# ChristophReich1996/Multi-StyleGAN

Measured on AMD Instinct MI355X. Metric: training images/sec (G+D step, 256^2, seq=3x2ch), higher is better.
Workload: dtype bf16

## Files before the change

### multi_stylegan_amd/csrc/conv_upconv.hip

```cpp
#include "conv_dispatch.h"
#include <stdlib.h>

typedef __bf16 bf16v8 __attribute__((ext_vector_type(8)));
typedef const __attribute__((address_space(1))) char* gptr_t;
typedef __attribute__((address_space(3))) char* lds_t;

struct UpconvParams {
    int B, H, W, Cx, N, O, ldy;
    long long x_bstride, w_bstride, y_bstride;
    int m_tiles, xcd_samples;
};

constexpr int UC_M = 128, UC_K = 512, UC_ROW = UC_K * 2;
constexpr int UC_PATCH = 32 * 64 * 2;

constexpr int UC_WAVES = 8;

__global__ __launch_bounds__(64 * UC_WAVES, 1) void conv_upconv_kernel(const bf16_t* __restrict__ x, const bf16_t* __restrict__ w,
                                                             bf16_t* __restrict__ y, UpconvParams p) {
    __shared__ __attribute__((aligned(16))) char smem[UC_M * UC_ROW + UC_WAVES * UC_PATCH];
    const int tid = threadIdx.x, lane = tid & 63, wid = tid >> 6;
    const int wid_u = __builtin_amdgcn_readfirstlane(wid);
    const int lr = lane & 31, lh = lane >> 5;
    int b, tile;
    if (p.xcd_samples) {
        const int xcd = blockIdx.x & 7, k = blockIdx.x >> 3;
        const int j = k / p.m_tiles;
        tile = k - j * p.m_tiles;
        b = xcd + 8 * j;
    } else {
        b = blockIdx.x / p.m_tiles;
        tile = blockIdx.x - b * p.m_tiles;
    }
    b = __builtin_amdgcn_readfirstlane(b);
    tile = __builtin_amdgcn_readfirstlane(tile);
    const int m0 = tile * UC_M;
    const int hw = p.H * p.W;

    {
        const gptr_t xb = (gptr_t)(x + (long long)b * p.x_bstride);
#pragma unroll 4
        for (int j = 0; j < UC_M / UC_WAVES; ++j) {
            const int r = wid_u * (UC_M / UC_WAVES) + j;
            const int m = m0 + r < hw ? m0 + r : 0;
            const gptr_t src = xb + ((long long)m * p.Cx + ((lane ^ (r & 15)) << 3)) * 2;
            __builtin_amdgcn_global_load_lds(src, (lds_t)(smem + r * UC_ROW), 16, 0, 0);
        }
        asm volatile("s_waitcnt vmcnt(0)" ::: "memory");
        __syncthreads();
    }

    const bf16_t* wb = w + (long long)b * p.w_bstride;
    bf16_t* yb = y + (long long)b * p.y_bstride;
    char* patch = smem + UC_M * UC_ROW + wid * UC_PATCH;
    const int swz = lr & 15;
    const int n_slices = p.N / 64;

    for (int slice = wid_u; slice < n_slices; slice += UC_WAVES) {
        const int n0 = slice * 64;
        f32x16 acc[4][2];
#pragma unroll
        for (int i = 0; i < 4; ++i)
#pragma unroll
            for (int j = 0; j < 2; ++j)
#pragma unroll
                for (int e = 0; e < 16; ++e) acc[i][j][e] = 0.f;

        const bf16_t* wrow[2] = {wb + (long long)(n0 + lr) * UC_K + 32 * lh, wb + (long long)(n0 + 32 + lr) * UC_K + 32 * lh};
        bf16v8 fb[2][2][4];
#pragma unroll
        for (int j = 0; j < 2; ++j)
#pragma unroll
            for (int u = 0; u < 4; ++u) fb[0][j][u] = *reinterpret_cast<const bf16v8*>(wrow[j] + 8 * u);
        bf16v8 fa[4];
        auto read_a = [&](int step, int i) __attribute__((always_inline)) {
            const int slot = ((8 * (step >> 2) + 4 * lh + (step & 3)) ^ swz) << 4;
            fa[i] = *reinterpret_cast<const bf16v8*>(smem + (32 * i + lr) * UC_ROW + slot);
        };
#pragma unroll
        for (int i = 0; i < 4; ++i) read_a(0, i);
#pragma unroll
        for (int t = 0; t < UC_K / 64; ++t) {
            if (t + 1 < UC_K / 64) {
#pragma unroll
                for (int j = 0; j < 2; ++j)
#pragma unroll
                    for (int u = 0; u < 4; ++u)
// ... 18 lines not shown
#pragma unroll
        for (int i = 0; i < 4; ++i) {
#pragma unroll
            for (int j = 0; j < 2; ++j)
#pragma unroll
                for (int g = 0; g < 4; ++g) {
                    const int unit = 8 * j + 2 * g + lh;
                    uint2 pk;
                    pk.x = (unsigned)f2bf(acc[i][j][4 * g + 0]) | ((unsigned)f2bf(acc[i][j][4 * g + 1]) << 16);
                    pk.y = (unsigned)f2bf(acc[i][j][4 * g + 2]) | ((unsigned)f2bf(acc[i][j][4 * g + 3]) << 16);
                    *reinterpret_cast<uint2*>(patch + lr * 128 + ((unit ^ (lr & 15)) << 3)) = pk;
                }
            asm volatile("s_waitcnt lgkmcnt(0)" ::: "memory");
            u32x4 v[4];
#pragma unroll
            for (int pass = 0; pass < 4; ++pass) {
                const int row = pass * 8 + er;
                v[pass] = *reinterpret_cast<const u32x4*>(patch + row * 128 + ((ec ^ ((row & 15) >> 1)) << 4));
                if (row & 1) v[pass] = u32x4{v[pass][2], v[pass][3], v[pass][0], v[pass][1]};
            }
#pragma unroll
            for (int pass = 0; pass < 4; ++pass) {
                const int m = m0 + 32 * i + pass * 8 + er;
                if (m < hw) {
                    const int oh = m / p.W, ow = m - oh * p.W;
                    const long long pix = (long long)(2 * oh + dy) * (2 * p.W) + 2 * ow + dx;
                    *reinterpret_cast<u32x4*>(yb + pix * p.ldy + c0 + ec * 8) = v[pass];
                }
            }
            asm volatile("s_waitcnt lgkmcnt(0)" ::: "memory");
        }
    }
}

bool conv_upconv_eligible(const ConvProblem& q, const ActEpilogue* act, bool has_bias, ConvPlan* plan) {
    static const int enabled = msg_tunable("MSG_CONV_UPCONV", 1);
    if (q.dtype != MSG_BF16 || has_bias || conv_act_mode(act)) return false;
    if (!enabled || !q.pixel_shuffle || !q.per_sample() || q.kh != 1 || q.kw != 1 || q.stride != 1 || q.pad != 0 || q.in_up != 1)
        return false;
    if (q.Cx != UC_K || q.Ck != UC_K || q.N % 256 || (q.N / 4) % 64 || q.IH != q.OH || q.IW != q.OW) return false;
    const long long hw = (long long)q.OH * q.OW, m_tiles = (hw + UC_M - 1) / UC_M;
    if (hw < 16384 || hw >= (1ll << 30)) return false;
    if (m_tiles * q.B < 256 || m_tiles * q.B >= (1ll << 31)) return false;
    if (q.w_batch_stride < (long long)q.N * UC_K) return false;
    *plan = ConvPlan{CONV_UPCONV, UC_M, q.N, true};
    return true;
}

void conv_upconv_launch(const ConvProblem& q, const ConvPlan&, const void* x, const void* w, void* y, void* stream) {
    UpconvParams p{};
    p.B = q.B; p.H = q.OH; p.W = q.OW; p.Cx = q.Cx; p.N = q.N; p.O = q.N / 4; p.ldy = q.ldy;
    p.x_bstride = q.x_bstride();
    p.w_bstride = q.w_batch_stride;
    p.y_bstride = q.y_bstride();
    p.m_tiles = (int)(((long long)q.OH * q.OW + UC_M - 1) / UC_M);
    static const int xcd_order = msg_tunable("MSG_UPCONV_XCD", 1);
    p.xcd_samples = xcd_order && q.B % 8 == 0;
    dim3 grid((unsigned)((long long)p.m_tiles * q.B));
    hipLaunchKernelGGL(conv_upconv_kernel, grid, dim3(64 * UC_WAVES), 0, (hipStream_t)stream, (const bf16_t*)x, (const bf16_t*)w,
                       (bf16_t*)y, p);
}
```

### include/msg_hip.h

```cpp
#ifndef MSG_HIP_H
#define MSG_HIP_H

#ifdef __cplusplus
extern "C" {
#endif

enum { MSG_OK = 0, MSG_EINVAL = -1, MSG_EUNSUPPORTED = -2, MSG_ELAUNCH = -3 };
enum { MSG_F32 = 0, MSG_BF16 = 1, MSG_F16 = 2, MSG_F64 = 3, MSG_F32_SPLIT = 4 };

#define MSG_ABI_VERSION 5
int msg_abi_version(void);
const char* msg_build_arch(void);
const char* msg_strerror(int code);

int msg_upfirdn2d(const void* x, const float* fir, void* y, int dtype,
                  int major, int in_h, int in_w, int minor, int kh, int kw,
                  int up_x, int up_y, int down_x, int down_y,
                  int pad_x0, int pad_x1, int pad_y0, int pad_y1, void* stream);

int msg_upfirdn2d_pitched(const void* x, const float* fir, void* y, int dtype,
                          int major, int in_h, int in_w, int minor, int in_pitch, int kh, int kw,
                          int up_x, int up_y, int down_x, int down_y,
                          int pad_x0, int pad_x1, int pad_y0, int pad_y1, void* stream);

// ... 155 lines not shown
long long msg_act_pointwise_head_backward_workspace(long long npix, int C);
int msg_act_pointwise_head_backward(const void* x, const float* bias, const float* w, const float* gy, void* gx,
                                    float* grad_bias_and_w, int dtype, long long npix, int C, float wscale,
                                    float alpha, float scale, float* ws, long long ws_floats, void* stream);

int msg_linear_fprop(const float* x, const float* w, const float* bias, float* y, int M, int N, int K,
                     float gain, float bias_gain, void* stream);
int msg_linear_dgrad(const float* gy, const float* w, float* gx, int M, int N, int K, float gain, void* stream);
int msg_linear_wgrad(const float* gy, const float* x, float* gw, float* gb, int M, int N, int K,
                     float gain, float bias_gain, void* stream);

int msg_linear_grouped_fprop(const float* x, const int* slot, const float* const* w, const float* const* bias, float* y,
                             int G, int M, int N, int K, int L, float gain, float bias_gain, void* stream);
int msg_linear_grouped_dgrad(const float* gy, const float* const* w, float* gx, int G, int M, int N, int K, float gain,
                             void* stream);
int msg_linear_grouped_wgrad(const float* gy, const float* x, const int* slot, float* gw, float* gb, int G, int M, int N,
                             int K, int L, float gain, float bias_gain, void* stream);
int msg_linear_grouped_wgrad_ptrs(const float* gy, const float* x, const int* slot, float* const* gw, float* const* gb, int G,
                                  int M, int N, int K, int L, float gain, float bias_gain, void* stream);

enum {
    MSG_PLAN_REG = 0,
    MSG_PLAN_DMA = 1,
    MSG_PLAN_PP = 2,
    MSG_PLAN_ROW3 = 3,
    MSG_PLAN_ROW3N = 4,
    MSG_PLAN_THIN = 5,
    MSG_PLAN_UPCONV = 6,
    MSG_FPLAN_FIELDS = 5
};
int msg_conv2d_fprop_launch_plan(int dtype, int B, int IH, int IW, int Cx, int Ck, int OH, int OW, int N, int ldy,
                                 int kh, int kw, int stride, int pad, int in_up, int pixel_shuffle,
                                 long long w_batch_stride, int has_bias, int epilogue, long long* out, int n_out_fields);
enum {
    MSG_WPLAN_GENERIC = 0,
    MSG_WPLAN_DMA = 1,
    MSG_WPLAN_UNI = 2,
    MSG_WPLAN_ROW3 = 3,
    MSG_WPLAN_ROW3_W32 = 4,
    MSG_WPLAN_FIELDS = 11
};
int msg_conv2d_wgrad_plan(int dtype, int B, int IH, int IW, int Cx, int I, int OH, int OW, int ldgy,
                          int O, int ldgw, int kh, int kw, int stride, int pad, int pixel_shuffle,
                          int per_sample, int k_chunks, long long* out, int n_out_fields);
int msg_conv2d_fprop_plan(int dtype, int B, int IH, int IW, int Cx, int Ck, int OH, int OW, int N,
                          int kh, int kw, long long w_batch_stride);
long long msg_conv2d_fprop_act_backward_workspace(int dtype, int B, int IH, int IW, int Cx, int Ck, int OH, int OW,
                                                  int N, int kh, int kw, long long w_batch_stride, int has_noise);
int msg_conv2d_fprop_upconv_eligible(int B, int IH, int IW, int Cx, int Ck, int OH, int OW, int N, int kh, int kw,
                                     int stride, int pad, int in_up, int pixel_shuffle, long long w_batch_stride);
int msg_conv2d_fprop_thin_eligible(int B, int IH, int IW, int Cx, int Ck, int OH, int OW, int N, int ldy, int kh, int kw,
                                   int stride, int pad, int in_up, int pixel_shuffle, int act_mode);

int msg_flat_adam(float* param, const float* grad, float* exp_avg, float* exp_avg_sq, float* ema, long long n,
                  const float* coef, float lr, float beta1, float beta2, float eps, int step, float ema_decay,
                  void* stream);
int msg_flat_ema(float* ema, const float* param, long long n, float decay, void* stream);

long long msg_tlfm_prepare_workspace(int B, int T);
int msg_tlfm_prepare(const unsigned short* raw, const unsigned char* hflip, void* out, int dtype,
                     int B, int C, int T, int H, int W, int vflip,
                     float lo1, float div1, float lo2, float div2,
                     unsigned int* ws, void* stream);

int msg_tlfm_frame_range(const unsigned short* frames, long long N, int H, int W,
                         unsigned int* range, void* stream);
// ... 34 lines not shown
```

### multi_stylegan_amd/csrc/conv_fprop.hip

```cpp
#include "conv_dispatch.h"
#include <stdlib.h>

typedef __bf16 bf16v8 __attribute__((ext_vector_type(8)));
typedef const __attribute__((address_space(1))) char* gptr_t;
typedef const __attribute__((address_space(1))) u32x4* gvec_t;
typedef __attribute__((address_space(3))) char* lds_t;

struct ConvParams {
    int B, IH, IW, Cx, Ck, OH, OW, N, ldy;
    int kh, kw, stride, pad, in_up, pixel_shuffle, per_sample;
    long long x_bstride, w_bstride, y_bstride;
    int Mtot, n_chunks, n_iters, m_tiles, n_tiles;
    ActEpilogue act;
};

constexpr int BM = 128, BN = 128, ROWB = 128;
constexpr int STAGE_BYTES = (BM + BN) * ROWB;
__device__ __attribute__((aligned(256))) unsigned int g_zero_page[16384];

__device__ __forceinline__ int swz(int row, int slot) { return row * ROWB + ((slot ^ ((row >> 1) & 7)) << 4); }

template <int SPLIT>
__device__ __forceinline__ void split_park(const u32x4& raw, char* dst) {
    uint2 pl[3];
#pragma unroll
    for (int h = 0; h < 2; ++h) {
        const float x0 = __uint_as_float(raw[2 * h]), x1 = __uint_as_float(raw[2 * h + 1]);
        const unsigned hp = (unsigned)f2bf(x0) | ((unsigned)f2bf(x1) << 16);
        const float r0 = x0 - __uint_as_float(hp << 16), r1 = x1 - __uint_as_float(hp & 0xffff0000u);
        const unsigned mp = (unsigned)f2bf(r0) | ((unsigned)f2bf(r1) << 16);
        (h ? pl[0].y : pl[0].x) = hp;
        (h ? pl[1].y : pl[1].x) = mp;
        if constexpr (SPLIT == 3) {
            const float q0 = r0 - __uint_as_float(mp << 16), q1 = r1 - __uint_as_float(mp & 0xffff0000u);
            (h ? pl[2].y : pl[2].x) = (unsigned)f2bf(q0) | ((unsigned)f2bf(q1) << 16);
        }
    }
#pragma unroll
    for (int p = 0; p < SPLIT; ++p) *reinterpret_cast<uint2*>(dst + p * 64) = pl[p];
}

template <typename T, bool DMA, int LEAN = 0, int SPLIT = 0>
__global__ __launch_bounds__(256, LEAN ? LEAN : 2) void conv_fprop_kernel(const T* __restrict__ x, const T* __restrict__ w,
                                                            T* __restrict__ y, const float* __restrict__ bias,
                                                            ConvParams p) {
    constexpr int VEC = 16 / sizeof(T);
    constexpr int BKE = ROWB / sizeof(T);
    static_assert(!LEAN || (!DMA && sizeof(T) == 2), "lean variant: bf16, register staging");
    static_assert(SPLIT == 0 || sizeof(T) == 4, "split-bf16 products are a mode of the fp32-storage kernel");
    static_assert(SPLIT == 0 || !DMA, "the split planes are written from the staging registers");
    constexpr int SROW = SPLIT ? SPLIT * 64 + 16 : ROWB;
    constexpr int STAGE = SPLIT ? (BM + BN) * SROW : STAGE_BYTES;
    constexpr bool ONE_STAGE = LEAN != 0 || SPLIT == 3;
    constexpr int SMEM_BYTES = ONE_STAGE ? (STAGE > 65536 || sizeof(T) == 2 ? STAGE : 65536) : 2 * STAGE;
    __shared__ __attribute__((aligned(16))) char smem[SMEM_BYTES];

    const int tid = threadIdx.x, lane = tid & 63, wid = tid >> 6;
    const int wm = wid >> 1, wn = wid & 1;
    const int lr = lane & 31, lh = lane >> 5;
    const unsigned L = xcd_remap(blockIdx.x, gridDim.x);
    const int n0 = (int)(L % p.n_tiles) * BN;
    const int m0 = (int)(L / p.n_tiles) * BM;
    const int bz = blockIdx.z;

    const int wid_u = __builtin_amdgcn_readfirstlane(wid);
    const int slot_phys = tid & 7;
    int row_of[4];
#pragma unroll
    for (int j = 0; j < 4; ++j) row_of[j] = DMA ? (wid * 32 + 8 * j + (lane >> 3)) : ((tid >> 3) + 32 * j);
    const int slot = DMA ? 0 : slot_phys;
    int a_ih0[4], a_iw0[4];
    long long a_boff[4];
    int a_slot[4];
    bool a_ok[4];
    const int ohw = p.OH * p.OW;
#pragma unroll
    for (int j = 0; j < 4; ++j) {
        const int m = m0 + row_of[j];
        const int slot_j = DMA ? (slot_phys ^ ((row_of[j] >> 1) & 7)) : slot_phys;
        a_ok[j] = m < p.Mtot;
        const int mm = a_ok[j] ? m : 0;
        const int b = p.per_sample ? bz : mm / ohw;
        const int pix = p.per_sample ? mm : mm - b * ohw;
        const int oh = pix / p.OW, ow = pix - oh * p.OW;
        a_ih0[j] = oh * p.stride - p.pad;
        a_iw0[j] = ow * p.stride - p.pad;
        a_boff[j] = ((long long)((DMA && p.per_sample) ? 0 : b) * p.x_bstride + slot_j * VEC +
// ... 158 lines not shown
                        for (int order = SPLIT - 1; order >= 0; --order)
#pragma unroll
                            for (int pa = 0; pa <= order; ++pa)
                                acc[i][j] = __builtin_amdgcn_mfma_f32_32x32x16_bf16(bf[order - pa][j], af[pa][i], acc[i][j], 0, 0, 0);
                    }
            }
        } else {
#pragma unroll
            for (int q = 0; q < 4; ++q) {
                f32x4 fa[2], fb[2];
#pragma unroll
                for (int t = 0; t < 2; ++t) {
                    fa[t] = *reinterpret_cast<const f32x4*>(sa + swz(wm * 64 + t * 32 + lr, 4 * lh + q));
                    fb[t] = *reinterpret_cast<const f32x4*>(sb + swz(wn * 64 + t * 32 + lr, 4 * lh + q));
                }
#pragma unroll
                for (int e = 0; e < 4; ++e)
#pragma unroll
                    for (int i = 0; i < 2; ++i)
#pragma unroll
                        for (int j = 0; j < 2; ++j)
                            acc[i][j] = __builtin_amdgcn_mfma_f32_32x32x2f32(fb[j][e], fa[i][e], acc[i][j], 0, 0, 0);
            }
        }
    };
    if constexpr (ONE_STAGE) {
        load_next();
        for (int it = 0; it < p.n_iters; ++it) {
            if (it) __syncthreads();
            park(0);
            if (it + 1 < p.n_iters) load_next();
            __syncthreads();
            mma_step(smem);
        }
    } else {
        if constexpr (DMA) {
            dma_stage = 0;
            load_next();
        } else {
            load_next();
            park(0);
            if (p.n_iters > 1) load_next();
        }
        for (int it = 0; it < p.n_iters; ++it) {
            if constexpr (DMA) asm volatile("s_waitcnt vmcnt(0)" ::: "memory");
            __syncthreads();
            if constexpr (DMA) {
                if (it + 1 < p.n_iters) { dma_stage = (it + 1) & 1; load_next(); }
            } else {
                if (it + 1 < p.n_iters) park((it + 1) & 1);
                if (it + 2 < p.n_iters) load_next();
            }
            mma_step(smem + (it & 1) * STAGE);
        }
    }
    if constexpr (DMA) asm volatile("s_waitcnt vmcnt(0)" ::: "memory");
    __syncthreads();

    constexpr int PITCH = 64 * sizeof(T);
    constexpr int UNITB = 4 * sizeof(T);
    char* ep = smem + wid * (64 * PITCH);
#pragma unroll
    for (int j = 0; j < 2; ++j)
#pragma unroll
        for (int g = 0; g < 4; ++g) {
            const int unit = 8 * j + 2 * g + lh;
// ... 83 lines not shown
    }
    T* ybase = y + (p.pixel_shuffle ? nn : n);
    if (n_ok && lim >= VEC) {
#pragma unroll
        for (int pass = 0; pass < NPASS; ++pass)
            if (gp[pass] >= 0) *reinterpret_cast<u32x4*>(ybase + (long long)gp[pass] * p.ldy) = v[pass];
    } else if (n_ok) {
#pragma unroll
        for (int pass = 0; pass < NPASS; ++pass) {
            if (gp[pass] < 0) continue;
            T tmp[VEC];
            *reinterpret_cast<u32x4*>(tmp) = v[pass];
            T* dst = ybase + (long long)gp[pass] * p.ldy;
            for (int e = 0; e < lim; ++e) dst[e] = tmp[e];
        }
    }
}

static ConvPlan conv_generic_select(const ConvProblem& q) {
    const int n_iters = q.kh * q.kw * (q.Ck / (ROWB / q.esz()));
    static const int variant = msg_tunable("MSG_CONV_VARIANT", 0);
    const bool dma = q.fits31() && (variant == 1 || (variant == 0 && n_iters >= 8));
    static const int lean_max = msg_tunable("MSG_CONV_LEAN", 4);
    ConvPlan plan{CONV_REG, BM, BN, true};
    if (q.split) plan.kernel = CONV_REG_SPLIT;
    else if (dma) plan.kernel = CONV_DMA;
    else if (q.dtype == MSG_BF16 && n_iters <= lean_max) plan.kernel = CONV_REG_LEAN;
    const long long mtot = q.mtot(), blocks = ((mtot + BM - 1) / BM) * ((q.N + BN - 1) / BN);
    plan.supported = mtot < (1ll << 31) && blocks < (1ll << 31) &&
                     (long long)(n_iters + 1) * ROWB + 128 <= 65536;
    return plan;
}

static void conv_generic_launch(const ConvProblem& q, const ConvPlan& plan, const void* x, const void* w, const float* bias, void* y,
                                const ActEpilogue* act, void* stream) {
    ConvParams p{};
    conv_fill_common(p, q, act);
    conv_fill_taps(p, q);
    p.n_chunks = q.Ck / (ROWB / q.esz());
    p.n_iters = q.kh * q.kw * p.n_chunks;
    p.m_tiles = (int)((q.mtot() + BM - 1) / BM);
    p.n_tiles = (q.N + BN - 1) / BN;
    dim3 grid((unsigned)((long long)p.m_tiles * p.n_tiles), 1, q.samples());
#define GENERIC(T, ...) hipLaunchKernelGGL((conv_fprop_kernel<T, __VA_ARGS__>), grid, dim3(256), 0, (hipStream_t)stream, \
                                           (const T*)x, (const T*)w, (T*)y, bias, p)
    const bool bf16 = q.dtype == MSG_BF16;
    if (bf16 && plan.kernel == CONV_REG_LEAN) GENERIC(bf16_t, false, 3);
    else if (bf16 && plan.kernel == CONV_DMA) GENERIC(bf16_t, true);
    else if (bf16) GENERIC(bf16_t, false);
    else if (plan.kernel == CONV_REG_SPLIT) GENERIC(float, false, 0, 3);
    else if (plan.kernel == CONV_DMA) GENERIC(float, true);
    else GENERIC(float, false);
#undef GENERIC
}

ConvPlan conv_fprop_select(const ConvProblem& q, const ActEpilogue* act, bool has_bias) {
    ConvPlan plan;
    if (conv_thin_eligible(q, act, &plan)) return plan;
    if (conv_upconv_eligible(q, act, has_bias, &plan)) return plan;
    if (conv_row3_eligible(q, act, has_bias, &plan)) return plan;
    if (conv_pp_eligible(q, &plan)) return plan;
    return conv_generic_select(q);
}

static ConvProblem conv_problem(int dtype, int B, int IH, int IW, int Cx, int Ck, int OH, int OW, int N, int ldy,
                                int kh, int kw, int stride, int pad, int in_up, int pixel_shuffle, long long w_batch_stride) {
    const int split = dtype == MSG_F32_SPLIT ? 3 : 0;
    return ConvProblem{split ? (int)MSG_F32 : dtype, split, B, IH, IW, Cx, Ck, OH, OW, N, ldy, kh, kw, stride, pad, in_up, pixel_shuffle,
                       w_batch_stride};
}

static ConvPlan fprop_select(const ConvProblem& q, int act_mode, bool has_bias) {
    ActEpilogue act{};
    act.enabled = act_mode;
    return conv_fprop_select(q, &act, has_bias);
}

static int fprop_check(const ConvProblem& q, const void* const* io) {
    if (q.B < 0 || q.IH <= 0 || q.IW <= 0 || q.OH <= 0 || q.OW <= 0 || q.N <= 0 || q.kh <= 0 || q.kw <= 0 || q.stride <= 0 ||
        q.in_up <= 0 || q.Cx <= 0 || q.Ck <= 0 || q.ldy <= 0 || (io && (!io[0] || !io[1] || !io[2])))
        return MSG_EINVAL;
    if (q.dtype != MSG_F32 && q.dtype != MSG_BF16) return MSG_EUNSUPPORTED;
    const int vec = 16 / q.esz(), bke = ROWB / q.esz();
// ... 49 lines not shown
    for (int k = 0; k < MSG_FPLAN_FIELDS && k < n_out_fields; ++k) out[k] = fields[k];
    return MSG_OK;
}

static ConvProblem conv_query_problem(int dtype, int B, int IH, int IW, int Cx, int Ck, int OH, int OW, int N, int kh, int kw,
                                      long long w_batch_stride) {
    return conv_problem(dtype, B, IH, IW, Cx, Ck, OH, OW, N, N <= 8 ? 8 : (N + 7) / 8 * 8, kh, kw, 1, kh / 2, 1, 0, w_batch_stride);
}
extern "C" int msg_conv2d_fprop_plan(int dtype, int B, int IH, int IW, int Cx, int Ck, int OH, int OW, int N,
                                     int kh, int kw, long long w_batch_stride) {
    return plan_code(fprop_select(conv_query_problem(dtype, B, IH, IW, Cx, Ck, OH, OW, N, kh, kw, w_batch_stride), 0, false).kernel);
}
extern "C" long long msg_conv2d_fprop_act_backward_workspace(int dtype, int B, int IH, int IW, int Cx, int Ck, int OH, int OW,
                                                             int N, int kh, int kw, long long w_batch_stride, int has_noise) {
    const ConvProblem q = conv_query_problem(dtype, B, IH, IW, Cx, Ck, OH, OW, N, kh, kw, w_batch_stride);
    long long rows, entries;
    act_backward_partials(q, fprop_select(q, 3, false), &rows, &entries);
    return rows ? rows * N + (has_noise ? entries : 0) : 0;
}
extern "C" int msg_conv2d_fprop_upconv_eligible(int B, int IH, int IW, int Cx, int Ck, int OH, int OW, int N, int kh, int kw,
                                                int stride, int pad, int in_up, int pixel_shuffle, long long w_batch_stride) {
    return fprop_select(conv_problem(MSG_BF16, B, IH, IW, Cx, Ck, OH, OW, N, N / 4, kh, kw, stride, pad, in_up, pixel_shuffle,
                                     w_batch_stride), 0, false).kernel == CONV_UPCONV;
}
extern "C" int msg_conv2d_fprop_thin_eligible(int B, int IH, int IW, int Cx, int Ck, int OH, int OW, int N, int ldy,
                                              int kh, int kw, int stride, int pad, int in_up, int pixel_shuffle,
                                              int act_mode) {
    const ConvKernel kernel = fprop_select(conv_problem(MSG_BF16, B, IH, IW, Cx, Ck, OH, OW, N, ldy, kh, kw, stride, pad, in_up,
                                                        pixel_shuffle, 0), act_mode, false).kernel;
    return kernel == CONV_THIN_N ? 1 : kernel == CONV_THIN_K ? 2 : 0;
}

static int conv2d_fprop_impl(const void* x, const void* w, const float* bias, void* y, const ConvProblem& q,
                             const ActEpilogue& act, void* stream) {
    const void* const io[3] = {x, w, y};
    ConvPlan plan;
    const int rc = fprop_plan_for(q, act.enabled, bias != nullptr, io, &plan);
    if (rc != MSG_OK || q.B == 0) return rc;
    if (act.mask && !is_row3(plan)) return MSG_EUNSUPPORTED;
    switch (plan.kernel) {
        case CONV_THIN_N: case CONV_THIN_K: conv_thin_launch(q, plan, x, w, bias, y, &act, stream); break;
        case CONV_UPCONV: conv_upconv_launch(q, plan, x, w, y, stream); break;
        case CONV_ROW3: case CONV_ROW3N: conv_row3_launch(q, plan, x, w, bias, y, &act, stream); break;
        case CONV_PP: conv_pp_launch(q, plan, x, w, bias, y, &act, stream); break;
        case CONV_DMA: case CONV_REG: case CONV_REG_LEAN: case CONV_REG_SPLIT:
            conv_generic_launch(q, plan, x, w, bias, y, &act, stream); break;
    }
    return MSG_CHECK_LAUNCH();
}

extern "C" int msg_conv2d_fprop(const void* x, const void* w, const float* bias, void* y, int dtype,
                                int B, int IH, int IW, int Cx, int Ck, int OH, int OW, int N, int ldy,
                                int kh, int kw, int stride, int pad, int in_up, int pixel_shuffle,
                                long long w_batch_stride, void* stream) {
    ActEpilogue act{};
    return conv2d_fprop_impl(x, w, bias, y, conv_problem(dtype, B, IH, IW, Cx, Ck, OH, OW, N, ldy, kh, kw, stride, pad, in_up,
                                                         pixel_shuffle, w_batch_stride), act, stream);
}

extern "C" int msg_conv2d_fprop_act_mask(const void* x, const void* w, void* y, int dtype,
                                         int B, int IH, int IW, int Cx, int Ck, int OH, int OW, int N, int ldy,
                                         int kh, int kw, int stride, int pad, long long w_batch_stride,
                                         const float* act_bias, const float* noise, const float* noise_weight,
                                         int noise_batch, float alpha, float scale, unsigned char* mask, void* stream) {
    if (noise && (!noise_weight || (noise_batch != 1 && noise_batch != B))) return MSG_EINVAL;
    ActEpilogue act{act_bias, noise, noise_weight, noise_batch, 1, alpha, scale, nullptr, 0, 0.f, mask};
    return conv2d_fprop_impl(x, w, nullptr, y, conv_problem(dtype, B, IH, IW, Cx, Ck, OH, OW, N, ldy, kh, kw, stride, pad, 1, 0,
                                                            w_batch_stride), act, stream);
}

extern "C" int msg_conv2d_fprop_act(const void* x, const void* w, void* y, int dtype,
                                    int B, int IH, int IW, int Cx, int Ck, int OH, int OW, int N, int ldy,
                                    int kh, int kw, int stride, int pad, long long w_batch_stride,
                                    const float* act_bias, const float* noise, const float* noise_weight,
                                    int noise_batch, float alpha, float scale, void* stream) {
    return msg_conv2d_fprop_act_mask(x, w, y, dtype, B, IH, IW, Cx, Ck, OH, OW, N, ldy, kh, kw, stride, pad, w_batch_stride,
                                     act_bias, noise, noise_weight, noise_batch, alpha, scale, nullptr, stream);
}

extern "C" int msg_conv2d_fprop_residual(const void* x, const void* w, void* y, int dtype,
                                         int B, int IH, int IW, int Cx, int Ck, int OH, int OW, int N, int ldy,
// ... 49 lines not shown
```

Before: 156.9.

## Split upconv waves into MFMA producer and store consumer roles

Restructures the pixel-shuffle upconv kernel so four waves only run MFMA GEMM slices and four waves only drain results. Accumulators pass through LDS patch ring buffers synchronised by workgroup-scope acquire/release flags, so global stores overlap with compute. It also prefetches the next slice's weights across slice boundaries and precomputes the output offsets. The cost is half as many waves issuing MFMA, spin-wait overhead on the flags, and more complex scheduling. The old symmetric kernel is kept only under MSG_TUNING.

```diff
diff --git a/multi_stylegan_amd/csrc/conv_upconv.hip b/multi_stylegan_amd/csrc/conv_upconv.hip
--- a/multi_stylegan_amd/csrc/conv_upconv.hip
+++ b/multi_stylegan_amd/csrc/conv_upconv.hip
@@ -15,14 +15,11 @@
 constexpr int UC_PATCH = 32 * 64 * 2;
 
 constexpr int UC_WAVES = 8;
-
-__global__ __launch_bounds__(64 * UC_WAVES, 1) void conv_upconv_kernel(const bf16_t* __restrict__ x, const bf16_t* __restrict__ w,
-                                                             bf16_t* __restrict__ y, UpconvParams p) {
-    __shared__ __attribute__((aligned(16))) char smem[UC_M * UC_ROW + UC_WAVES * UC_PATCH];
-    const int tid = threadIdx.x, lane = tid & 63, wid = tid >> 6;
-    const int wid_u = __builtin_amdgcn_readfirstlane(wid);
-    const int lr = lane & 31, lh = lane >> 5;
-    int b, tile;
+constexpr int UC_TILE = UC_M * UC_ROW;
+constexpr int UC_LDS = UC_TILE + UC_WAVES * UC_PATCH;
+
+__device__ __forceinline__ void uc_prologue(char* smem, const bf16_t* __restrict__ x, const UpconvParams& p, int lane, int wid_u,
+                                            int& b, int& tile) {
     if (p.xcd_samples) {
         const int xcd = blockIdx.x & 7, k = blockIdx.x >> 3;
         const int j = k / p.m_tiles;
@@ -36,23 +33,33 @@
     tile = __builtin_amdgcn_readfirstlane(tile);
     const int m0 = tile * UC_M;
     const int hw = p.H * p.W;
-
-    {
-        const gptr_t xb = (gptr_t)(x + (long long)b * p.x_bstride);
+    const gptr_t xb = (gptr_t)(x + (long long)b * p.x_bstride);
 #pragma unroll 4
-        for (int j = 0; j < UC_M / UC_WAVES; ++j) {
-            const int r = wid_u * (UC_M / UC_WAVES) + j;
-            const int m = m0 + r < hw ? m0 + r : 0;
-            const gptr_t src = xb + ((long long)m * p.Cx + ((lane ^ (r & 15)) << 3)) * 2;
-            __builtin_amdgcn_global_load_lds(src, (lds_t)(smem + r * UC_ROW), 16, 0, 0);
-        }
-        asm volatile("s_waitcnt vmcnt(0)" ::: "memory");
-        __syncthreads();
-    }
+    for (int j = 0; j < UC_M / UC_WAVES; ++j) {
+        const int r = wid_u * (UC_M / UC_WAVES) + j;
+        const int m = m0 + r < hw ? m0 + r : 0;
+        const gptr_t src = xb + ((long long)m * p.Cx + ((lane ^ (r & 15)) << 3)) * 2;
+        __builtin_amdgcn_global_load_lds(src, (lds_t)(smem + r * UC_ROW), 16, 0, 0);
+    }
+    asm volatile("s_waitcnt vmcnt(0)" ::: "memory");
+    __syncthreads();
+}
+
+#ifdef MSG_TUNING
+__global__ __launch_bounds__(64 * UC_WAVES, 1) void conv_upconv_sym_kernel(const bf16_t* __restrict__ x, const bf16_t* __restrict__ w,
+                                                                 bf16_t* __restrict__ y, UpconvParams p) {
+    __shared__ __attribute__((aligned(16))) char smem[UC_LDS];
+    const int tid = threadIdx.x, lane = tid & 63, wid = tid >> 6;
+    const int wid_u = __builtin_amdgcn_readfirstlane(wid);
+    const int lr = lane & 31, lh = lane >> 5;
+    int b, tile;
+    uc_prologue(smem, x, p, lane, wid_u, b, tile);
+    const int m0 = tile * UC_M;
+    const int hw = p.H * p.W;
 
     const bf16_t* wb = w + (long long)b * p.w_bstride;
     bf16_t* yb = y + (long long)b * p.y_bstride;
-    char* patch = smem + UC_M * UC_ROW + wid * UC_PATCH;
+    char* patch = smem + UC_TILE + wid * UC_PATCH;
     const int swz = lr & 15;
     const int n_slices = p.N / 64;
 
@@ -137,6 +144,179 @@
         }
     }
 }
+
+#endif
+
+constexpr int UC_CWAVES = 4;
+constexpr int UC_FLAGS = UC_TILE + 7 * UC_PATCH;
+
+__device__ __forceinline__ unsigned uc_flag_load(const unsigned* f) {
+    return __hip_atomic_load(f, __ATOMIC_ACQUIRE, __HIP_MEMORY_SCOPE_WORKGROUP);
+}
+__device__ __forceinline__ void uc_flag_store(unsigned* f, unsigned v) {
+    __hip_atomic_store(f, v, __ATOMIC_RELEASE, __HIP_MEMORY_SCOPE_WORKGROUP);
+}
+
+__global__ __launch_bounds__(64 * UC_WAVES, 1) void conv_upconv_kernel(const bf16_t* __restrict__ x, const bf16_t* __restrict__ w,
+                                                             bf16_t* __restrict__ y, UpconvParams p) {
+    __shared__ __attribute__((aligned(16))) char smem[UC_LDS];
+    const int tid = threadIdx.x, lane = tid & 63, wid = tid >> 6;
+    const int wid_u = __builtin_amdgcn_readfirstlane(wid);
+    const int lr = lane & 31, lh = lane >> 5;
+    if (tid < 2 * UC_CWAVES) reinterpret_cast<unsigned*>(smem + UC_FLAGS)[tid] = 0;
+    int b, tile;
+    uc_prologue(smem, x, p, lane, wid_u, b, tile);
+    const int m0 = tile * UC_M;
+    const int hw = p.H * p.W;
+    const int n_slices = p.N / 64;
+
+    const int c = wid_u & (UC_CWAVES - 1);
+    const int ring = c < 3 ? 2 : 1;
+    char* const pbase = smem + UC_TILE + c * 2 * UC_PATCH;
+    unsigned* const flags = reinterpret_cast<unsigned*>(smem + UC_FLAGS) + 2 * c;
+    unsigned n = 0;
+
+    if (wid_u < UC_CWAVES) {
+        const bf16_t* wb = w + (long long)b * p.w_bstride + (long long)lr * UC_K + 32 * lh;
+        const int swz = lr & 15;
+        bf16v8 fb[2][2][4];
+#pragma unroll
+        for (int j = 0; j < 2; ++j)
+#pragma unroll
+            for (int u = 0; u < 4; ++u)
+                fb[0][j][u] = *reinterpret_cast<const bf16v8*>(wb + (long long)(c * 64 + 32 * j) * UC_K + 8 * u);
+        bf16v8 fa[4];
+        int abase[8];
+#pragma unroll
+        for (int k = 0; k < 8; ++k) abase[k] = lr * UC_ROW + ((((k & 3) | ((k >> 2) << 3) | (4 * lh)) ^ swz) << 4);
+        auto read_a = [&](int step, int i, int r) __attribute__((always_inline)) {
+            fa[r] = *reinterpret_cast<const bf16v8*>(smem + abase[step & 7] + (step >> 3) * 256 + 32 * i * UC_ROW);
+        };
+        f32x16 acc[4][2];
+        auto hand_over = [&](int i) __attribute__((always_inline)) {
+            uint2 pk[2][4];
+#pragma unroll
+            for (int j = 0; j < 2; ++j)
+#pragma unroll
+                for (int g = 0; g < 4; ++g) {
+                    pk[j][g].x = (unsigned)f2bf(acc[i][j][4 * g + 0]) | ((unsigned)f2bf(acc[i][j][4 * g + 1]) << 16);
+                    pk[j][g].y = (unsigned)f2bf(acc[i][j][4 * g + 2]) | ((unsigned)f2bf(acc[i][j][4 * g + 3]) << 16);
+                }
+            const unsigned slot = n & (unsigned)(ring - 1);
+            char* patch = pbase + slot * UC_PATCH;
+            while (__builtin_amdgcn_readfirstlane(uc_flag_load(flags + slot)) != 0) __builtin_amdgcn_s_sleep(1);
+#pragma unroll
+            for (int j = 0; j < 2; ++j)
+#pragma unroll
+                for (int g = 0; g < 4; ++g) {
+                    const int unit = 8 * j + 2 * g + lh;
+                    *reinterpret_cast<uint2*>(patch + lr * 128 + ((unit ^ (lr & 15)) << 3)) = pk[j][g];
+                }
+            ++n;
+            uc_flag_store(flags + slot, n);
+        };
+#pragma unroll
+        for (int u = 0; u < 4; ++u) read_a(u, 0, u);
+        bool first = true;
+        for (int slice = c; slice < n_slices; slice += UC_CWAVES) {
+            const bf16_t* wrow = wb + (long long)slice * 64 * UC_K;
+            const bool more = slice + UC_CWAVES < n_slices;
+#pragma unroll
+            for (int t = 0; t < UC_K / 64; ++t) {
+                if (t + 1 < UC_K / 64) {
+#pragma unroll
+                    for (int j = 0; j < 2; ++j)
+#pragma unroll
+                        for (int u = 0; u < 4; ++u)
+                            fb[(t + 1) & 1][j][u] = *reinterpret_cast<const bf16v8*>(wrow + 32 * j * UC_K + 64 * (t + 1) + 8 * u);
+                } else if (more) {
+#pragma unroll
+                    for (int j = 0; j < 2; ++j)
+#pragma unroll
+                        for (int u = 0; u < 4; ++u)
+                            fb[0][j][u] = *reinterpret_cast<const bf16v8*>(wrow + (long long)(64 * UC_CWAVES + 32 * j) * UC_K + 8 * u);
+                }
+                __builtin_amdgcn_sched_barrier(0);
+                if (t == 0) {
+#pragma unroll
+                    for (int i = 0; i < 4; ++i) {
+                        if (!first) hand_over(i);
+#pragma unroll
+                        for (int j = 0; j < 2; ++j)
+#pragma unroll
+                            for (int e = 0; e < 16; ++e) acc[i][j][e] = 0.f;
+#pragma unroll
+                        for (int u = 0; u < 4; ++u) {
+#pragma unroll
+                            for (int j = 0; j < 2; ++j)
+                                acc[i][j] = __builtin_amdgcn_mfma_f32_32x32x16_bf16(fb[0][j][u], fa[u], acc[i][j], 0, 0, 0);
+                            if (i < 3) read_a(u, i + 1, u);
+                            else read_a(4, u, u);
+                            __builtin_amdgcn_sched_barrier(0);
+                        }
+                    }
+                    first = false;
+                } else {
+#pragma unroll
+                    for (int u = 0; u < 4; ++u) {
+                        const int step = 4 * t + u;
+#pragma unroll
+                        for (int i = 0; i < 4; ++i) {
+#pragma unroll
+                            for (int j = 0; j < 2; ++j)
+                                acc[i][j] = __builtin_amdgcn_mfma_f32_32x32x16_bf16(fb[t & 1][j][u], fa[i], acc[i][j], 0, 0, 0);
+                            if (step + 1 < UC_K / 16) read_a(step + 1, i, i);
+                            else read_a(i, 0, i);
+                            __builtin_amdgcn_sched_barrier(0);
+                        }
+                    }
+                }
+            }
+        }
+        if (!first) {
+#pragma unroll
+            for (int i = 0; i < 4; ++i) hand_over(i);
+        }
+    } else {
+        bf16_t* yb = y + (long long)b * p.y_bstride;
+        const int er = lane >> 3, ec = lane & 7;
+        long long off[4][4];
+#pragma unroll
+        for (int i = 0; i < 4; ++i)
+#pragma unroll
+            for (int pass = 0; pass < 4; ++pass) {
+                const int m = m0 + 32 * i + pass * 8 + er;
+                const int oh = m / p.W, ow = m - oh * p.W;
+                off[i][pass] = m < hw ? ((long long)(2 * oh) * (2 * p.W) + 2 * ow) * p.ldy + ec * 8 : -1;
+            }
+        for (int slice = c; slice < n_slices; slice += UC_CWAVES) {
+            const int n0 = slice * 64;
+            const int q = n0 / p.O, c0 = n0 - q * p.O;
+            const int dy = q >> 1, dx = q & 1;
+            bf16_t* ys = yb + ((long long)dy * (2 * p.W) + dx) * p.ldy + c0;
+#pragma unroll
+            for (int i = 0; i < 4; ++i) {
+                const unsigned slot = n & (unsigned)(ring - 1);
+                const char* patch = pbase + slot * UC_PATCH;
+                ++n;
+                while (__builtin_amdgcn_readfirstlane(uc_flag_load(flags + slot)) != n) __builtin_amdgcn_s_sleep(1);
+                u32x4 v[4];
+#pragma unroll
+                for (int pass = 0; pass < 4; ++pass) {
+                    const int row = pass * 8 + er;
+                    v[pass] = *reinterpret_cast<const u32x4*>(patch + row * 128 + ((ec ^ ((row & 15) >> 1)) << 4));
+                }
+                uc_flag_store(flags + slot, 0);
+#pragma unroll
+                for (int pass = 0; pass < 4; ++pass) {
+                    if (er & 1) v[pass] = u32x4{v[pass][2], v[pass][3], v[pass][0], v[pass][1]};
+                    if (off[i][pass] >= 0) *reinterpret_cast<u32x4*>(ys + off[i][pass]) = v[pass];
+                }
+            }
+        }
+    }
+}
+
 
 bool conv_upconv_eligible(const ConvProblem& q, const ActEpilogue* act, bool has_bias, ConvPlan* plan) {
     static const int enabled = msg_tunable("MSG_CONV_UPCONV", 1);
@@ -162,6 +342,14 @@
     static const int xcd_order = msg_tunable("MSG_UPCONV_XCD", 1);
     p.xcd_samples = xcd_order && q.B % 8 == 0;
     dim3 grid((unsigned)((long long)p.m_tiles * q.B));
+#ifdef MSG_TUNING
+    static const int roles = msg_tunable("MSG_UPCONV_ROLES", 1);
+    if (!roles) {
+        hipLaunchKernelGGL(conv_upconv_sym_kernel, grid, dim3(64 * UC_WAVES), 0, (hipStream_t)stream, (const bf16_t*)x,
+                           (const bf16_t*)w, (bf16_t*)y, p);
+        return;
+    }
+#endif
     hipLaunchKernelGGL(conv_upconv_kernel, grid, dim3(64 * UC_WAVES), 0, (hipStream_t)stream, (const bf16_t*)x, (const bf16_t*)w,
                        (bf16_t*)y, p);
 }
```

Result: no change. 157.4 (median of 6 runs) (+0.3%).

## Rewrite upconv kernel with register-stationary activations and LDS weight ring pipeline

Applied to the files above, without the earlier changes.

Replaces the upconv GEMM kernel so each wave keeps its activation rows in registers and streams weight tiles through an 8-slot LDS ring. Loads use buffer DMA issued several stages ahead, and the two wave halves are skewed by four stages. Each column's epilogue is interleaved with the next column's MFMAs, and outputs are written with nontemporal stores. The aim is to stop re-reading weights from global memory per wave and to overlap loads with compute, at the cost of much more complex hand-scheduled barrier and waitcnt logic. The old kernel remains only as a tuning fallback.

```diff
diff --git a/multi_stylegan_amd/csrc/conv_upconv.hip b/multi_stylegan_amd/csrc/conv_upconv.hip
--- a/multi_stylegan_amd/csrc/conv_upconv.hip
+++ b/multi_stylegan_amd/csrc/conv_upconv.hip
@@ -15,8 +15,193 @@
 constexpr int UC_PATCH = 32 * 64 * 2;
 
 constexpr int UC_WAVES = 8;
+constexpr int UC_STAGE_ROW = 128, UC_STAGE = 128 * UC_STAGE_ROW;
+constexpr int UC_SLOTS = 8, UC_RING = UC_SLOTS * UC_STAGE;
+constexpr int UC_AHEAD = UC_SLOTS - 1;
+constexpr int UC_SKEW = 4;
 
 __global__ __launch_bounds__(64 * UC_WAVES, 1) void conv_upconv_kernel(const bf16_t* __restrict__ x, const bf16_t* __restrict__ w,
+                                                             bf16_t* __restrict__ y, UpconvParams p) {
+    __shared__ __attribute__((aligned(16))) char smem[UC_RING + UC_WAVES * UC_PATCH];
+    const int tid = threadIdx.x, lane = tid & 63, wid = tid >> 6;
+    const int wid_u = __builtin_amdgcn_readfirstlane(wid);
+    const int lr = lane & 31, lh = lane >> 5;
+    const int pg = wid_u & 3, h = wid_u >> 2;
+    int b, tile;
+    if (p.xcd_samples) {
+        const int xcd = blockIdx.x & 7, k = blockIdx.x >> 3;
+        const int j = k / p.m_tiles;
+        tile = k - j * p.m_tiles;
+        b = xcd + 8 * j;
+    } else {
+        b = blockIdx.x / p.m_tiles;
+        tile = blockIdx.x - b * p.m_tiles;
+    }
+    b = __builtin_amdgcn_readfirstlane(b);
+    tile = __builtin_amdgcn_readfirstlane(tile);
+    const int m0 = tile * UC_M;
+    const int hw = p.H * p.W;
+
+    const bf16_t* wb = w + (long long)b * p.w_bstride;
+    bf16_t* yb = y + (long long)b * p.y_bstride;
+    const int n_cols = p.N / 128;
+    const int n_stages = 8 * n_cols;
+
+    const msg_desc_t wdesc = msg_make_desc(wb);
+    const unsigned lds0 = (unsigned)(unsigned long long)(lds_t)smem;
+    int voff[2];
+#pragma unroll
+    for (int i = 0; i < 2; ++i) {
+        const int r = 16 * pg + 8 * i + (lane >> 3);
+        voff[i] = (64 * h + r) * UC_ROW + (((lane & 7) ^ ((r >> 1) & 7)) << 4);
+    }
+    auto dma_stage = [&](int g, int slot) __attribute__((always_inline)) {
+        const int s = g - UC_SKEW * h;
+        const bool live = s >= 0 && s < n_stages;
+        const int soff = live ? (s >> 3) * (128 * UC_ROW) + (s & 7) * UC_STAGE_ROW : 0;
+#pragma unroll
+        for (int i = 0; i < 2; ++i)
+            msg_dma16(wdesc, lds0 + slot * UC_STAGE + (64 * h + 16 * pg + 8 * i) * UC_STAGE_ROW, live ? voff[i] : MSG_DMA_OOB, soff);
+    };
+
+    bf16v8 xa[8][4];
+    {
+        const int m = m0 + 32 * pg + lr < hw ? m0 + 32 * pg + lr : 0;
+        const bf16_t* xr = x + (long long)b * p.x_bstride + (long long)m * p.Cx + 32 * lh;
+#pragma unroll
+        for (int P = 0; P < 8; ++P)
+#pragma unroll
+            for (int u = 0; u < 4; ++u)
+                xa[P][u] = *reinterpret_cast<const bf16v8*>(xr + 64 * ((P + UC_SKEW * h) & 7) + 8 * u);
+    }
+#pragma unroll
+    for (int g = 0; g < UC_AHEAD; ++g) dma_stage(g, g);
+
+    int foff[4];
+#pragma unroll
+    for (int u = 0; u < 4; ++u) foff[u] = (64 * h + lr) * UC_STAGE_ROW + (((4 * lh + u) ^ ((lr >> 1) & 7)) << 4);
+    bf16v8 fb[2][4];
+    auto read_f = [&](int slot, int j, int u) __attribute__((always_inline)) {
+        fb[j][u] = *reinterpret_cast<const bf16v8*>(smem + slot * UC_STAGE + j * 32 * UC_STAGE_ROW + foff[u]);
+    };
+    f32x16 acc[2];
+    auto stage = [&](int g, auto p_tag, auto first_tag) __attribute__((always_inline)) {
+        constexpr int P = decltype(p_tag)::value;
+        constexpr bool FIRST = decltype(first_tag)::value;
+#pragma unroll
+        for (int u = 0; u < 4; ++u)
+#pragma unroll
+            for (int j = 0; j < 2; ++j) {
+#if defined(__HIP_DEVICE_COMPILE__)
+                if (FIRST && u == 0) asm("v_mfma_f32_32x32x16_bf16 %0, %1, %2, 0" : "+v"(acc[j]) : "v"(fb[j][u]), "v"(xa[P][u]));
+                else asm("v_mfma_f32_32x32x16_bf16 %0, %1, %2, %0" : "+v"(acc[j]) : "v"(fb[j][u]), "v"(xa[P][u]));
+#endif
+                read_f((P + 1) & 7, j, u);
+                if (u == 0 && j == 1) dma_stage(g + UC_AHEAD, (P + UC_AHEAD) & 7);
+                __builtin_amdgcn_sched_barrier(0);
+            }
+    };
+    auto reads_only = [&](auto p_tag) __attribute__((always_inline)) {
+        constexpr int P = decltype(p_tag)::value;
+#pragma unroll
+        for (int u = 0; u < 4; ++u)
+#pragma unroll
+            for (int j = 0; j < 2; ++j) read_f((P + 1) & 7, j, u);
+    };
+    auto hand_over = [&](int g, int P) __attribute__((always_inline)) {
+        asm volatile("s_waitcnt vmcnt(%0)" :: "n"(2 * (UC_AHEAD - 2)) : "memory");
+        __builtin_amdgcn_sched_barrier(0);
+        asm volatile("s_barrier" ::: "memory");
+        __builtin_amdgcn_sched_barrier(0);
+    };
+    auto idle_period = [&](int g, int P) __attribute__((always_inline)) {
+        hand_over(g, P);
+        dma_stage(g + UC_AHEAD, (P + UC_AHEAD) & 7);
+    };
+    auto epilogue = [&](int col) __attribute__((always_inline)) {
+        const int n0 = 128 * col + 64 * h;
+        const int q = n0 / p.O, c0 = n0 - q * p.O;
+        const int dy = q >> 1, dx = q & 1;
+        int el = lane;
+        asm volatile("" : "+v"(el));
+        const int elr = el & 31, elh = el >> 5, er = el >> 3, ec = el & 7;
+        char* const epatch = smem + UC_RING + wid_u * UC_PATCH;
+        asm volatile("s_nop 7\n\ts_nop 7" ::: "memory");
+        __builtin_amdgcn_sched_barrier(0);
+#pragma unroll
+        for (int j = 0; j < 2; ++j)
+#pragma unroll
+            for (int g = 0; g < 4; ++g) {
+                const int unit = 8 * j + 2 * g + elh;
+                uint2 pk;
+                pk.x = (unsigned)f2bf(acc[j][4 * g + 0]) | ((unsigned)f2bf(acc[j][4 * g + 1]) << 16);
+                pk.y = (unsigned)f2bf(acc[j][4 * g + 2]) | ((unsigned)f2bf(acc[j][4 * g + 3]) << 16);
+                *reinterpret_cast<uint2*>(epatch + elr * 128 + ((unit ^ (elr & 15)) << 3)) = pk;
+            }
+        asm volatile("s_waitcnt lgkmcnt(0)" ::: "memory");
+        u32x4 v[4];
+#pragma unroll
+        for (int pass = 0; pass < 4; ++pass) {
+            const int row = pass * 8 + er;
+            v[pass] = *reinterpret_cast<const u32x4*>(epatch + row * 128 + ((ec ^ ((row & 15) >> 1)) << 4));
+            if (row & 1) v[pass] = u32x4{v[pass][2], v[pass][3], v[pass][0], v[pass][1]};
+        }
+#pragma unroll
+        for (int pass = 0; pass < 4; ++pass) {
+            const int m = m0 + 32 * pg + pass * 8 + er;
+            if (m < hw) {
+                const int oh = m / p.W, ow = m - oh * p.W;
+                const long long pix = (long long)(2 * oh + dy) * (2 * p.W) + 2 * ow + dx;
+                __builtin_nontemporal_store(v[pass], reinterpret_cast<u32x4*>(yb + pix * p.ldy + c0 + ec * 8));
+            }
+        }
+    };
+
+    __builtin_amdgcn_s_waitcnt(0x0f70);
+    __builtin_amdgcn_sched_barrier(0);
+    asm volatile("s_barrier" ::: "memory");
+    __builtin_amdgcn_sched_barrier(0);
+
+    using std::integral_constant;
+    constexpr integral_constant<bool, true> first{};
+    constexpr integral_constant<bool, false> later{};
+#define UC_STAGE_AT(g_, P_, first_) do { hand_over((g_), P_); stage((g_), integral_constant<int, P_>{}, first_); } while (0)
+    if (h == 0) {
+#pragma unroll
+        for (int u = 0; u < 4; ++u)
+#pragma unroll
+            for (int j = 0; j < 2; ++j) read_f(0, j, u);
+        for (int c = 0; c < n_cols; ++c) {
+            const int g = 8 * c;
+            hand_over(g, 0);
+            if (c > 0) epilogue(c - 1);
+            stage(g, integral_constant<int, 0>{}, first);
+            UC_STAGE_AT(g + 1, 1, later); UC_STAGE_AT(g + 2, 2, later); UC_STAGE_AT(g + 3, 3, later); UC_STAGE_AT(g + 4, 4, later);
+            UC_STAGE_AT(g + 5, 5, later); UC_STAGE_AT(g + 6, 6, later); UC_STAGE_AT(g + 7, 7, later);
+        }
+        idle_period(n_stages, 0);
+        epilogue(n_cols - 1);
+        idle_period(n_stages + 1, 1); idle_period(n_stages + 2, 2); idle_period(n_stages + 3, 3); idle_period(n_stages + 4, 4);
+    } else {
+        idle_period(0, 0); idle_period(1, 1); idle_period(2, 2); idle_period(3, 3);
+        reads_only(integral_constant<int, 3>{});
+        for (int c = 0; c < n_cols; ++c) {
+            const int g = 8 * c;
+            hand_over(g + 4, 4);
+            if (c > 0) epilogue(c - 1);
+            stage(g + 4, integral_constant<int, 4>{}, first);
+            UC_STAGE_AT(g + 5, 5, later); UC_STAGE_AT(g + 6, 6, later); UC_STAGE_AT(g + 7, 7, later);
+            UC_STAGE_AT(g + 8, 0, later); UC_STAGE_AT(g + 9, 1, later); UC_STAGE_AT(g + 10, 2, later); UC_STAGE_AT(g + 11, 3, later);
+        }
+        idle_period(n_stages + 4, 4);
+        epilogue(n_cols - 1);
+    }
+#undef UC_STAGE_AT
+    asm volatile("s_waitcnt vmcnt(0)" ::: "memory");
+}
+
+#ifdef MSG_TUNING
+__global__ __launch_bounds__(64 * UC_WAVES, 1) void conv_upconv_stationary_kernel(const bf16_t* __restrict__ x, const bf16_t* __restrict__ w,
                                                              bf16_t* __restrict__ y, UpconvParams p) {
     __shared__ __attribute__((aligned(16))) char smem[UC_M * UC_ROW + UC_WAVES * UC_PATCH];
     const int tid = threadIdx.x, lane = tid & 63, wid = tid >> 6;
@@ -137,6 +322,7 @@
         }
     }
 }
+#endif
 
 bool conv_upconv_eligible(const ConvProblem& q, const ActEpilogue* act, bool has_bias, ConvPlan* plan) {
     static const int enabled = msg_tunable("MSG_CONV_UPCONV", 1);
@@ -148,6 +334,7 @@
     if (hw < 16384 || hw >= (1ll << 30)) return false;
     if (m_tiles * q.B < 256 || m_tiles * q.B >= (1ll << 31)) return false;
     if (q.w_batch_stride < (long long)q.N * UC_K) return false;
+    if ((long long)q.N * UC_ROW >= (1ll << 31)) return false;
     *plan = ConvPlan{CONV_UPCONV, UC_M, q.N, true};
     return true;
 }
@@ -162,6 +349,14 @@
     static const int xcd_order = msg_tunable("MSG_UPCONV_XCD", 1);
     p.xcd_samples = xcd_order && q.B % 8 == 0;
     dim3 grid((unsigned)((long long)p.m_tiles * q.B));
+#ifdef MSG_TUNING
+    const int ring = msg_tunable("MSG_UPCONV_RING", 1);
+    if (!ring) {
+        hipLaunchKernelGGL(conv_upconv_stationary_kernel, grid, dim3(64 * UC_WAVES), 0, (hipStream_t)stream, (const bf16_t*)x,
+                           (const bf16_t*)w, (bf16_t*)y, p);
+        return;
+    }
+#endif
     hipLaunchKernelGGL(conv_upconv_kernel, grid, dim3(64 * UC_WAVES), 0, (hipStream_t)stream, (const bf16_t*)x, (const bf16_t*)w,
                        (bf16_t*)y, p);
 }
```

New measurement: 157.4 before, 158.0 after (median of 4 runs). Within noise of the previous version (+0.3%).

## Add deeper LDS-DMA ring pipeline for under-occupied generic conv fprop

Applied to the files above, without the earlier changes.

Adds a 3- or 4-stage LDS ring buffer mode to the DMA generic conv forward kernel, using partial vmcnt waits so several tile loads stay in flight. It is selected automatically when the grid has no more blocks than one round of CUs, where occupancy is too low to hide latency through other blocks. The larger shared-memory footprint and launch bound of 1 reduce occupancy, and the hardcoded vmcnt counts assume a fixed number of loads per stage. Also exposes query and explicit-stage entry points.

```diff
diff --git a/include/msg_hip.h b/include/msg_hip.h
--- a/include/msg_hip.h
+++ b/include/msg_hip.h
@@ -211,6 +211,13 @@
 int msg_conv2d_fprop_launch_plan(int dtype, int B, int IH, int IW, int Cx, int Ck, int OH, int OW, int N, int ldy,
                                  int kh, int kw, int stride, int pad, int in_up, int pixel_shuffle,
                                  long long w_batch_stride, int has_bias, int epilogue, long long* out, int n_out_fields);
+int msg_conv2d_fprop_launch_stages(int dtype, int B, int IH, int IW, int Cx, int Ck, int OH, int OW, int N, int ldy,
+                                   int kh, int kw, int stride, int pad, int in_up, int pixel_shuffle,
+                                   long long w_batch_stride, int has_bias, int epilogue);
+int msg_conv2d_fprop_stages(const void* x, const void* w, const float* bias, void* y, int dtype,
+                            int B, int IH, int IW, int Cx, int Ck, int OH, int OW, int N, int ldy,
+                            int kh, int kw, int stride, int pad, int in_up, int pixel_shuffle,
+                            long long w_batch_stride, int stages, void* stream);
 enum {
     MSG_WPLAN_GENERIC = 0,
     MSG_WPLAN_DMA = 1,
diff --git a/multi_stylegan_amd/csrc/conv_fprop.hip b/multi_stylegan_amd/csrc/conv_fprop.hip
--- a/multi_stylegan_amd/csrc/conv_fprop.hip
+++ b/multi_stylegan_amd/csrc/conv_fprop.hip
@@ -1,5 +1,6 @@
 #include "conv_dispatch.h"
 #include <stdlib.h>
+#include <atomic>
 
 typedef __bf16 bf16v8 __attribute__((ext_vector_type(8)));
 typedef const __attribute__((address_space(1))) char* gptr_t;
@@ -40,19 +41,20 @@
     for (int p = 0; p < SPLIT; ++p) *reinterpret_cast<uint2*>(dst + p * 64) = pl[p];
 }
 
-template <typename T, bool DMA, int LEAN = 0, int SPLIT = 0>
-__global__ __launch_bounds__(256, LEAN ? LEAN : 2) void conv_fprop_kernel(const T* __restrict__ x, const T* __restrict__ w,
+template <typename T, bool DMA, int LEAN = 0, int SPLIT = 0, int STAGES = 2>
+__global__ __launch_bounds__(256, LEAN ? LEAN : (STAGES > 2 ? 1 : 2)) void conv_fprop_kernel(const T* __restrict__ x, const T* __restrict__ w,
                                                             T* __restrict__ y, const float* __restrict__ bias,
                                                             ConvParams p) {
     constexpr int VEC = 16 / sizeof(T);
     constexpr int BKE = ROWB / sizeof(T);
     static_assert(!LEAN || (!DMA && sizeof(T) == 2), "lean variant: bf16, register staging");
+    static_assert(STAGES == 2 || (DMA && STAGES >= 3 && STAGES <= 4), "the deeper ring is a mode of the LDS-DMA pipeline");
     static_assert(SPLIT == 0 || sizeof(T) == 4, "split-bf16 products are a mode of the fp32-storage kernel");
     static_assert(SPLIT == 0 || !DMA, "the split planes are written from the staging registers");
     constexpr int SROW = SPLIT ? SPLIT * 64 + 16 : ROWB;
     constexpr int STAGE = SPLIT ? (BM + BN) * SROW : STAGE_BYTES;
     constexpr bool ONE_STAGE = LEAN != 0 || SPLIT == 3;
-    constexpr int SMEM_BYTES = ONE_STAGE ? (STAGE > 65536 || sizeof(T) == 2 ? STAGE : 65536) : 2 * STAGE;
+    constexpr int SMEM_BYTES = ONE_STAGE ? (STAGE > 65536 || sizeof(T) == 2 ? STAGE : 65536) : STAGES * STAGE;
     __shared__ __attribute__((aligned(16))) char smem[SMEM_BYTES];
 
     const int tid = threadIdx.x, lane = tid & 63, wid = tid >> 6;
@@ -277,6 +279,24 @@
             if (it + 1 < p.n_iters) load_next();
             __syncthreads();
             mma_step(smem);
+        }
+    } else if constexpr (DMA && STAGES > 2) {
+        int wr = 0;
+        for (int s = 0; s < STAGES - 1 && s < p.n_iters; ++s) { dma_stage = wr; load_next(); ++wr; }
+        int rd = 0;
+        for (int it = 0; it < p.n_iters; ++it) {
+            const int younger = min(STAGES - 2, p.n_iters - 1 - it);
+            if (younger >= 2) asm volatile("s_waitcnt vmcnt(16)" ::: "memory");
+            else if (younger == 1) asm volatile("s_waitcnt vmcnt(8)" ::: "memory");
+            else asm volatile("s_waitcnt vmcnt(0)" ::: "memory");
+            __syncthreads();
+            if (it + STAGES - 1 < p.n_iters) {
+                dma_stage = wr;
+                load_next();
+                if (++wr == STAGES) wr = 0;
+            }
+            mma_step(smem + rd * STAGE);
+            if (++rd == STAGES) rd = 0;
         }
     } else {
         if constexpr (DMA) {
@@ -426,8 +446,29 @@
     return plan;
 }
 
+static int conv_device_cus() {
+    static std::atomic<int> cached[64];
+    int dev = 0;
+    if (hipGetDevice(&dev) != hipSuccess || dev < 0 || dev >= 64) { (void)hipGetLastError(); return 256; }
+    int cus = cached[dev].load(std::memory_order_relaxed);
+    if (cus > 0) return cus;
+    if (hipDeviceGetAttribute(&cus, hipDeviceAttributeMultiprocessorCount, dev) != hipSuccess || cus <= 0) {
+        (void)hipGetLastError();
+        cus = 256;
+    }
+    cached[dev].store(cus, std::memory_order_relaxed);
+    return cus;
+}
+
+static int conv_ring_stages(const ConvProblem& q, const ConvPlan& plan) {
+    if (plan.kernel != CONV_DMA) return 0;
+    static const int depth = msg_tunable("MSG_CONV_RING_DEPTH", 4), rounds = msg_tunable("MSG_CONV_RING_ROUNDS", 1);
+    const long long blocks = ((q.mtot() + BM - 1) / BM) * ((q.N + BN - 1) / BN) * q.samples();
+    return (depth == 3 || depth == 4) && blocks <= (long long)rounds * conv_device_cus() ? depth : 2;
+}
+
 static void conv_generic_launch(const ConvProblem& q, const ConvPlan& plan, const void* x, const void* w, const float* bias, void* y,
-                                const ActEpilogue* act, void* stream) {
+                                const ActEpilogue* act, void* stream, int stages) {
     ConvParams p{};
     conv_fill_common(p, q, act);
     conv_fill_taps(p, q);
@@ -440,9 +481,13 @@
                                            (const T*)x, (const T*)w, (T*)y, bias, p)
     const bool bf16 = q.dtype == MSG_BF16;
     if (bf16 && plan.kernel == CONV_REG_LEAN) GENERIC(bf16_t, false, 3);
+    else if (bf16 && plan.kernel == CONV_DMA && stages == 4) GENERIC(bf16_t, true, 0, 0, 4);
+    else if (bf16 && plan.kernel == CONV_DMA && stages == 3) GENERIC(bf16_t, true, 0, 0, 3);
     else if (bf16 && plan.kernel == CONV_DMA) GENERIC(bf16_t, true);
     else if (bf16) GENERIC(bf16_t, false);
     else if (plan.kernel == CONV_REG_SPLIT) GENERIC(float, false, 0, 3);
+    else if (plan.kernel == CONV_DMA && stages == 4) GENERIC(float, true, 0, 0, 4);
+    else if (plan.kernel == CONV_DMA && stages == 3) GENERIC(float, true, 0, 0, 3);
     else if (plan.kernel == CONV_DMA) GENERIC(float, true);
     else GENERIC(float, false);
 #undef GENERIC
@@ -558,11 +603,12 @@
 }
 
 static int conv2d_fprop_impl(const void* x, const void* w, const float* bias, void* y, const ConvProblem& q,
-                             const ActEpilogue& act, void* stream) {
+                             const ActEpilogue& act, void* stream, int stages = 0) {
     const void* const io[3] = {x, w, y};
     ConvPlan plan;
     const int rc = fprop_plan_for(q, act.enabled, bias != nullptr, io, &plan);
     if (rc != MSG_OK || q.B == 0) return rc;
+    if (stages && plan.kernel != CONV_DMA) return MSG_EUNSUPPORTED;
     if (act.mask && !is_row3(plan)) return MSG_EUNSUPPORTED;
     switch (plan.kernel) {
         case CONV_THIN_N: case CONV_THIN_K: conv_thin_launch(q, plan, x, w, bias, y, &act, stream); break;
@@ -570,9 +616,30 @@
         case CONV_ROW3: case CONV_ROW3N: conv_row3_launch(q, plan, x, w, bias, y, &act, stream); break;
         case CONV_PP: conv_pp_launch(q, plan, x, w, bias, y, &act, stream); break;
         case CONV_DMA: case CONV_REG: case CONV_REG_LEAN: case CONV_REG_SPLIT:
-            conv_generic_launch(q, plan, x, w, bias, y, &act, stream); break;
+            conv_generic_launch(q, plan, x, w, bias, y, &act, stream, stages ? stages : conv_ring_stages(q, plan)); break;
     }
     return MSG_CHECK_LAUNCH();
+}
+
+extern "C" int msg_conv2d_fprop_launch_stages(int dtype, int B, int IH, int IW, int Cx, int Ck, int OH, int OW, int N, int ldy,
+                                              int kh, int kw, int stride, int pad, int in_up, int pixel_shuffle,
+                                              long long w_batch_stride, int has_bias, int epilogue) {
+    if (epilogue < 0 || epilogue > 3 || (epilogue && (has_bias || in_up != 1 || pixel_shuffle))) return MSG_EINVAL;
+    const ConvProblem q = conv_problem(dtype, B, IH, IW, Cx, Ck, OH, OW, N, ldy, kh, kw, stride, pad, in_up, pixel_shuffle, w_batch_stride);
+    ConvPlan plan;
+    const int rc = fprop_plan_for(q, epilogue, has_bias != 0, nullptr, &plan);
+    if (rc != MSG_OK || q.B == 0) return rc;
+    return conv_ring_stages(q, plan);
+}
+
+extern "C" int msg_conv2d_fprop_stages(const void* x, const void* w, const float* bias, void* y, int dtype,
+                                       int B, int IH, int IW, int Cx, int Ck, int OH, int OW, int N, int ldy,
+                                       int kh, int kw, int stride, int pad, int in_up, int pixel_shuffle,
+                                       long long w_batch_stride, int stages, void* stream) {
+    if (stages < 2 || stages > 4) return MSG_EUNSUPPORTED;
+    ActEpilogue act{};
+    return conv2d_fprop_impl(x, w, bias, y, conv_problem(dtype, B, IH, IW, Cx, Ck, OH, OW, N, ldy, kh, kw, stride, pad, in_up,
+                                                         pixel_shuffle, w_batch_stride), act, stream, stages);
 }
 
 extern "C" int msg_conv2d_fprop(const void* x, const void* w, const float* bias, void* y, int dtype,
```

Result: no change. 156.7 before, 156.6 after (-0.0%).
